# yynps737/zero-latency-yolo

Hardware: AMD Instinct MI355X
Metric: frames_per_sec (higher is better)
Workload: dtype bf16; 1 GPU; YOLOv8-nano 416x416 batch=64 throughput path (BASELINE configs[2]), bf16; engines_per_gpu=3, weights=seeded synthetic (no real weights offline), graph=True, parallelism=single GPU

## Files before the change

### zero-latency-yolo_amd/csrc/engine.cpp

```cpp
#include "zly_internal.h"
#include "weights.h"

#include <algorithm>
#include <atomic>
#include <chrono>
#include <condition_variable>
#include <deque>
#include <map>
#include <mutex>
#include <string>
#include <thread>
#include <type_traits>
#include <vector>
#include <string.h>
#include <stdio.h>
#include <stdlib.h>

namespace zly {

static thread_local std::string g_last_error;

static int fail(int code, const std::string& msg) { g_last_error = msg; return code; }

#define HIP_TRY(expr, code)                                                                        \
// ... 216 lines not shown
    num("ZLY_STEM1_TW", &sw->stem1_tw);
    num("ZLY_STEM1_TH", &sw->stem1_th);
    sw->stem1_keep_tiles = on("ZLY_STEM1_TW") || on("ZLY_STEM1_TH") || on("ZLY_STEM1_BIG_TILES");
    num("ZLY_PAIR_MIN_TILES", &sw->pair_min_tiles);
    num("ZLY_PAIR_WIDTHS", &sw->pair_widths);
    auto num_nonempty = [&](const char* name, int* out) { const char* v = getenv(name); if (v && *v) *out = atoi(v); };
    num_nonempty("ZLY_STAGE_SLOTS", &sw->stage_slots);
    num_nonempty("ZLY_STAGE_MB", &sw->stage_mb);
    num_nonempty("ZLY_INFLIGHT", &sw->inflight);
    { int d = 0; num_nonempty("ZLY_D2H_STREAM", &d); sw->d2h_stream = d != 0; }
    num("ZLY_PROFILE_INNER", &sw->profile_inner);
    if (sw->profile_inner < 1) sw->profile_inner = 1;
#ifdef ZLY_DIAG
    if (const char* v = getenv("ZLY_ABLATE_SKIP")) sw->ablate = std::string(",") + v + ",";
#endif
    sw->no_stream = on("ZLY_NO_STREAM");
    sw->stream_ct2 = on("ZLY_STREAM_CT2");
    num("ZLY_STREAM_MAX_NK", &sw->stream_max_nk);
    num("ZLY_STREAM_MIN_GROUPS", &sw->stream_min_groups);
    num("ZLY_STREAM_WGS", &sw->stream_wgs);
    num("ZLY_WS1", &sw->ws1_mode);
    sw->ws1_no_dual = on("ZLY_WS1_NO_DUAL");
    num("ZLY_WS1_MIN_PX", &sw->ws1_min_px);
    sw->ws1_max_bytes = on("ZLY_WS1_MAX_BYTES");
    sw->no_ws = on("ZLY_NO_WS");
    sw->no_ws_s2 = on("ZLY_NO_WS_S2");
    sw->no_ws_s2_c32 = on("ZLY_NO_WS_S2_C32");
    sw->ws_rowt = on("ZLY_WS_ROWT");
    num("ZLY_WS_TPW1_MAXCT", &sw->ws_tpw1_maxct);
    num("ZLY_WS_MIN_TILES", &sw->ws_min_tiles);
    num("ZLY_WS_MAX_BYTES", &sw->ws_max_bytes);
    num("ZLY_WS_PAIR", &sw->ws_pair);
    num("ZLY_WS_PAIR_GRID", &sw->ws_pair_grid);
    num("ZLY_WS_PAIR_MAX_TILES", &sw->ws_pair_max_tiles);
    sw->no_wres = on("ZLY_NO_WRES");
    num("ZLY_WRES_MAXCHUNKS", &sw->wres_maxchunks);
    sw->lds_s2_pt1 = on("ZLY_LDS_S2_PT1");
    num("ZLY_LDS_MIN_TILES", &sw->lds_min_tiles);
    num("ZLY_LDS_WGS_PER_CU", &sw->lds_wgs_per_cu);
    num("ZLY_DIRECT_PT4_MIN", &sw->direct_pt4_min);
    num("ZLY_DIRECT_PT2_MIN", &sw->direct_pt2_min);
    num("ZLY_DIRECT_KSPLIT_NK", &sw->direct_ksplit_nk);
    num("ZLY_C2F32_NW", &sw->c2f32_nw);
    num("ZLY_C2F_LDS_KB", &sw->c2f_lds_kb);
    if (const char* ft = getenv("ZLY_C2F_TILE")) { int th = 0, tw = 0; if (sscanf(ft, "%d,%d", &th, &tw) == 2) { sw->c2f_tile_th = th; sw->c2f_tile_tw = tw; } }
    sw->c2f64 = on("ZLY_C2F64");
}

struct PlanBuilder {
    Plan* p;
    const ModelFile& model;
    const zly_config& cfg;
    const int dtype;
    const Switches& sw;
    const size_t esz;
    const int kstep;
    std::string err;

    bool bf16() const { return dtype == ZLY_DTYPE_BF16; }
    bool fail(const std::string& msg) { err = msg; return false; }
    int add_buffer(const std::string& name, int H, int W, int C, bool f32 = false) {
        Buffer b;
        b.name = name; b.H = H; b.W = W; b.C = C; b.f32 = f32;
        p->bufs.push_back(b);
        return (int)p->bufs.size() - 1;
    }
// ... 2139 lines not shown
    const Op& op = e->ops[(size_t)i];
    std::string k;
    switch (L.kind) {
    case LK_NONE:
        switch (t[(size_t)L.covered_by].kind) {
        case LK_STEM: case LK_STEM1: k = op.kind == OP_PREPROCESS ? "(fused into stem_fused_kernel)" : "(fused into the previous launch)"; break;
        case LK_PAIR: case LK_WS_PAIR: k = "(fused into the previous launch)"; break;
        case LK_C2F: k = "(fused into the C2f kernel at " + e->ops[(size_t)L.covered_by].name + ")"; break;
        case LK_SPPF_FUSED: k = "(fused into the SPPF kernel at model.9.cv1)"; break;
        case LK_MULTI: k = "(in a merged Detect launch)"; break;
        case LK_HEAD: k = op.kind == OP_CONV ? "(computed in the Detect tail at surviving anchors)" : "(covered by the last tail launch)"; break;
        }
        break;
    case LK_PREPROCESS: k = L.lb ? "preprocess_kernel<LB> (letterbox)" : "preprocess_kernel"; break;
    case LK_STEM: k = L.lb ? "stem_fused_kernel<LB> (letterbox)" : "stem_fused_kernel"; break;
    case LK_STEM1: k = L.lb ? "stem_model1_kernel<LB> (letterbox preprocess+model.0+model.1)" : "stem_model1_kernel (preprocess+model.0+model.1)"; break;
    case LK_SPPF_POOL: k = L.pool16 ? "sppf_pool16_kernel<DPP row windows, one barrier>" : "sppf_pool_kernel"; break;
    case LK_SPPF_FUSED: k = "sppf_fused_kernel<cv1+3 pools+cv2,SPLIT=" + std::to_string(sppf_split(e->ops[(size_t)e->sppf_cv2].cout, n, e->sw)) + ">"; break;
    case LK_MULTI: k = L.multi_ct == 3 ? "conv_igemm_multi_kernel<CT=3> (the 3 Detect stems)" : "conv_igemm_multi_kernel<CT=2> (the 6 Detect branch convs)"; break;
    case LK_C2F: {
        const C2fGroup& g = e->c2fs[(size_t)op.c2f];
        k = "c2f_kernel<C=" + std::to_string(g.c) + (g.c == 32 ? ",NW=" + std::to_string(L.c2f.nw) : std::string()) +
            (g.mode == 3 ? ",cv1+bottleneck+cv2>" : g.mode == 1 ? ",cv1+bottleneck>" : ",bottleneck+cv2>");
        break;
    }
    case LK_PAIR: k = "bottleneck_pair_kernel<" + std::to_string(e->pairs[(size_t)op.pair].c) + ">"; break;
    case LK_WS_PAIR: k = std::string("conv3x3_ws_pair_kernel<") + (e->pairs[(size_t)op.pair].res ? "RES," : "") + "64->64->64," + std::to_string(L.ws_pair.g.TH) + "x" + std::to_string(L.ws_pair.g.TW) + " tiles>"; break;
    case LK_CONV_WSK: k = "conv3x3_wsk_kernel<K=720 packed across taps,5 channel tiles>"; break;
    case LK_CONV: {
        const int cin = op.in.C + (op.in2.buf >= 0 ? op.in2.C : 0);
        const ConvPlan& c = L.conv;
        switch (c.kind) {
        case CONV_WS1: k = std::string("conv1x1_ws_kernel<") + (op.in2.buf >= 0 ? "dual-source," : "") + "NK=" + std::to_string(cin / 32) + "," + std::to_string(c.ct) + " channel tiles," + std::to_string(c.pt * 16) + " px>"; break;
        case CONV_WS: k = std::string("conv3x3_ws_kernel<") + (op.stride == 2 ? "S=2," : "") + (c.rowt ? "ROWT," : "") + (c.tpw1 ? "TPW=1," : "TPW=2,") + std::to_string(c.ct) + " channel tiles>"; break;
        case CONV_LDS: k = "conv3x3_lds_kernel<S=" + std::to_string(op.stride) + ",CT=" + std::to_string(c.ct) + ",PT=" + std::to_string(c.pt) + (c.wres ? ",wres>" : ">"); break;
        case CONV_STREAM: k = "conv1x1_stream_kernel<CT=" + std::to_string(c.ct) + ",PT=" + std::to_string(c.pt) + ",NK=" + std::to_string((cin + 31) / 32) + ">"; break;
        default: k = std::string("conv_igemm_kernel<") + (op.ks == 1 ? (op.in2.buf >= 0 ? "1x1 dual-source" : "1x1") : (c.fastk ? "3x3" : "3x3 generic-K")) +
                 ",CT=" + std::to_string(c.ct) + ",PT=" + std::to_string(c.pt) + ",KSPLIT=" + std::to_string(c.ksplit) + ">";
        }
        break;
    }
    case LK_HEAD: {
        k = L.lb ? "head_fused_kernel<LB> (letterbox box mapping)" : "head_fused_kernel";
        std::string lv;
        for (int l = 0; l < 3; ++l)
            if (L.box_mode[l] && (L.only_level < 0 || L.only_level == l)) lv += std::string(lv.empty() ? "" : ",") + "P" + std::to_string(3 + l) + (L.box_mode[l] == 1 ? ":ws" : ":lds");
        if (!lv.empty()) k += " (+ box conv in k-step order " + lv + ")";
        break;
    }
    case LK_NMS: k = "nms_kernel"; break;
    }
    snprintf(out, cap, "%s", k.c_str());
    return ZLY_OK;
}

int32_t zly_launch_info_at(zly_engine* e, int32_t i, int32_t n, zly_launch_info* out)
{
    if (!e || !out || i < 0 || i >= (int32_t)e->ops.size() || n < 1 || n > e->cfg.max_batch) return fail(ZLY_ERR_INVALID_ARGUMENT, "bad argument");
    std::lock_guard<std::mutex> lk(e->mu);
    memset(out, 0, sizeof *out);
    const int nops = (int)e->ops.size();
    const std::vector<Launch>& t = resolve_launches(e, n);
    out->covered_by = t[(size_t)i].covered_by;
    if (out->covered_by != i) return ZLY_OK;
    std::vector<char> in_group((size_t)nops, 0);
    for (int j = 0; j < nops; ++j) in_group[(size_t)j] = t[(size_t)j].covered_by == i ? 1 : 0;
    std::map<int, std::vector<char>> written_in, read_out, counted_in, counted_out;
// ... 117 lines not shown
```

### zero-latency-yolo_amd/csrc/kernels_conv.hip

```cpp
#include "zly_internal.h"
#include "conv_device.h"
#include <type_traits>
#include <algorithm>

namespace zly {

template <int CT>
__device__ __forceinline__ void load_bias(const ConvArgs& a, int tile0, int kq, f32x4 (&bias)[CT])
{
    const int ntiles = (a.Cout + 15) >> 4;
    const int paired = (ntiles >> 1) << 1;
#pragma unroll
    for (int c = 0; c < CT; ++c) {
        const int ch = tile_channel(tile0 + c, kq, paired);
        bias[c] = ch < a.Cout ? *reinterpret_cast<const f32x4*>(a.bias + ch) : f32x4{0.f, 0.f, 0.f, 0.f};
    }
}

template <typename T, int CT>
__device__ __forceinline__ void epilogue_px(const ConvArgs& a, f32x4 (&v)[CT], const f32x4 (&bias)[CT], int tile0, int kq, int m)
{
    const int ntiles = (a.Cout + 15) >> 4;
    const int paired = (ntiles >> 1) << 1;
    f32x4 o[CT];
// ... 685 lines not shown
        for (int k = 0; k < 5; ++k) o[k] = dsum[k];
        o[5] = ditems; o[6] = __builtin_amdgcn_s_memtime() - dstart; o[7] = dsum[5];
    }
#endif
}

typedef void (*conv_lds_fn)(const ConvArgs, int, int, int, int);

template <int S, int PT>
static conv_lds_fn pick_lds_ct(int ct) {
    switch (ct) {
        case 2: return conv3x3_lds_kernel<S, 2, PT>;
        case 3: return conv3x3_lds_kernel<S, 3, PT>;
        case 4: return conv3x3_lds_kernel<S, 4, PT>;
        case 5: return conv3x3_lds_kernel<S, 5, PT>;
    }
    return nullptr;
}
static conv_lds_fn pick_lds(int stride, int pt, int ct) {
    if (stride == 1) return pt == 1 ? pick_lds_ct<1, 1>(ct) : pt == 2 ? pick_lds_ct<1, 2>(ct) : pick_lds_ct<1, 4>(ct);
    return pt == 1 ? pick_lds_ct<2, 1>(ct) : pick_lds_ct<2, 2>(ct);
}
static size_t lds_bytes(int stride, int pt, int ct, int wchunks = 1) {
    size_t patch = 0;
    if (stride == 1) patch = pt == 1 ? LdsGeom<1, 1>::PATCH_BYTES : pt == 2 ? LdsGeom<1, 2>::PATCH_BYTES : LdsGeom<1, 4>::PATCH_BYTES;
    else             patch = pt == 1 ? LdsGeom<2, 1>::PATCH_BYTES : LdsGeom<2, 2>::PATCH_BYTES;
    return patch + (size_t)wchunks * 9 * ct * 1024;
}

#ifdef ZLY_WS_DIAG
__device__ unsigned long long* g_ws_diag = nullptr;
#endif

template <int TPW, int NKS, bool RES, bool ROWT = false, int S = 1>
__global__ __launch_bounds__(256, 2) void conv3x3_ws_kernel(const ConvArgs a, const WsGeom g)
{
    extern __shared__ __attribute__((aligned(16))) unsigned char smem[];
    unsigned char* lpatch = smem;
    const int PW = S == 1 ? g.TW + 8 : g.TW + 8 * ((g.TW + 8) / 8), PH = S == 1 ? g.TH + 2 : 2 * g.TH + 1;
    const int PWV = S == 1 ? g.TW + 2 : 2 * g.TW + 1;
    static_assert(S == 1 || !ROWT, "row tiles: stride 1");
    const int nthreads = blockDim.x;
    const int tid = threadIdx.x, lane = tid & 63;
    const int wave = __builtin_amdgcn_readfirstlane(tid >> 6);
    const int p = lane & 15, kq = lane >> 4;
    const int wc = wave % g.nwc, wp = wave / g.nwc;
    const int ntiles_c = (a.cout_pad + 15) >> 4;
    const bf16_t* __restrict__ in = static_cast<const bf16_t*>(a.in) + a.in_co;
    const int upp = a.Cin >> 3;
    const int NPU = PH * PW * upp;
    const float inv_upp = 1.0f / (float)upp, invPW = 1.0f / (float)PW, invTW = 1.0f / (float)g.TW;
    const int NPB = g.TH * g.TW, nct = ROWT ? g.TH : (NPB + 15) >> 4;
    const int tiles_per_img = g.tiles_x * g.tiles_y;

    bf16x8 w[TPW][NKS];
    {
        const bf16_t* __restrict__ wb = static_cast<const bf16_t*>(a.wgt) + lane * 8;
#pragma unroll
        for (int t = 0; t < TPW; ++t) {
            const int tile = min(wc * TPW + t, ntiles_c - 1);
#pragma unroll
            for (int s = 0; s < NKS; ++s) w[t][s] = *reinterpret_cast<const bf16x8*>(wb + ((size_t)tile * a.nk + s) * 512);
        }
    }
    f32x4 biasr[TPW];
    load_bias<TPW>(a, wc * TPW, kq, biasr);
    const __amdgpu_buffer_rsrc_t rout = __builtin_amdgcn_make_buffer_rsrc(a.out, 0, (unsigned)((size_t)a.M * a.out_cs * 2), 0x00020000);
    const __amdgpu_buffer_rsrc_t rres = __builtin_amdgcn_make_buffer_rsrc(const_cast<void*>(a.res ? a.res : a.out), 0,
                                                                          (unsigned)((size_t)a.M * (a.res ? a.res_cs : a.out_cs) * 2), 0x00020000);
    const int ch0 = TPW == 2 ? wc * 32 + kq * 8 : tile_channel(wc, kq, (((a.Cout + 15) >> 4) >> 1) << 1);
    constexpr bool has_res = RES;
    int toff[NKS];
#pragma unroll
    for (int s = 0; s < NKS; ++s) {
        const int tap = s / (NKS / 9), chunk = s - tap * (NKS / 9);
        const int ky = tap / 3, kx = tap - ky * 3;
        toff[s] = (ky * PW + kx) * g.pitch + chunk * 64;
    }
#ifdef ZLY_WS_DIAG
    unsigned long long dsum[4] = {0, 0, 0, 0}, dT0 = 0, dT1 = 0;
#define WSSTAMP(t) do { __builtin_amdgcn_sched_barrier(0); asm volatile("s_memtime %0\n\ts_waitcnt lgkmcnt(0)" : "=s"(t) :: "memory"); __builtin_amdgcn_sched_barrier(0); } while (0)
#define WSPHASE(k) do { WSSTAMP(dT1); dsum[k] += dT1 - dT0; dT0 = dT1; } while (0)
    const unsigned long long dstart = __builtin_amdgcn_s_memtime();
    WSSTAMP(dT0);
#else
#define WSPHASE(k) do { } while (0)
#endif

    const int upitch = g.pitch >> 4;
    const int NLU = PH * PW * upitch, ndma = (NLU + 63) >> 6;
    const float inv_upitch = 1.0f / (float)upitch;
    const int patch_bytes = ndma * 1024;
    const __amdgpu_buffer_rsrc_t rin = __builtin_amdgcn_make_buffer_rsrc(const_cast<bf16_t*>(in), 0, (unsigned)(((size_t)a.M / (a.Ho * a.Wo) * a.H * a.W * a.in_cs - a.in_co) * 2), 0x00020000);
    auto dma_patch = [&](int tl, unsigned char* dst) {
        const int b = tl / tiles_per_img;
        const int r = tl - b * tiles_per_img;
        const int ty = r / g.tiles_x;
        const int y0 = ty * g.TH, x0 = (r - ty * g.tiles_x) * g.TW;
        for (int k = wave; k < ndma; k += nthreads >> 6) {
            const int u = k * 64 + lane;
            const int px = (int)(((float)u + 0.5f) * inv_upitch), part = u - px * upitch;
            const int py = (int)(((float)px + 0.5f) * invPW), pxx = px - py * PW;
            const int gy = y0 * S - 1 + py, gx = x0 * S - 1 + pxx;
            const bool ok = part < upp && pxx < PWV && py < PH && (unsigned)gy < (unsigned)a.H && (unsigned)gx < (unsigned)a.W;
            const unsigned off = ok ? (unsigned)((((b * a.H + gy) * a.W + gx) * a.in_cs) * 2 + part * 16) : 0x80000000u;
            __builtin_amdgcn_raw_ptr_buffer_load_lds(rin, (__attribute__((address_space(3))) void*)(dst + k * 1024), 16, off, 0, 0, 0);
        }
    };
    (void)NPU; (void)inv_upp; (void)patch_bytes;
    if ((int)blockIdx.x < g.total_tiles) dma_patch(blockIdx.x, lpatch);
    for (int tl = blockIdx.x; tl < g.total_tiles; tl += gridDim.x) {
        const int b = tl / tiles_per_img;
        const int r = tl - b * tiles_per_img;
        const int ty = r / g.tiles_x;
        const int y0 = ty * g.TH, x0 = (r - ty * g.tiles_x) * g.TW;
        unsigned char* cur = lpatch;
        asm volatile("s_waitcnt vmcnt(0)" ::: "memory");
        __syncthreads();
        WSPHASE(0);
        auto pair_setup = [&](int t0, const unsigned char* (&px)[2], int (&ob)[2], int (&rb)[2]) {
#pragma unroll
            for (int h2 = 0; h2 < 2; ++h2) {
                const int t = min(t0 + h2 * g.nwp, nct - 1);
                const int q = ROWT ? (p < g.TW ? t * g.TW + p : NPB) : t * 16 + p;
                const int qc = min(q, NPB - 1);
                const int oy = ROWT ? t : (int)(((float)qc + 0.5f) * invTW), ox = ROWT ? p : qc - oy * g.TW;
                px[h2] = cur + (oy * S * PW + ox * S) * g.pitch + kq * 16;
                const int gy = y0 + oy, gx = x0 + ox;
                const bool ok = (t0 + h2 * g.nwp < nct) && q < NPB && gy < a.Ho && gx < a.Wo;
                const int m = (b * a.Ho + gy) * a.Wo + gx;
                ob[h2] = ok ? (m * a.out_cs + a.out_co + ch0) * 2 : (int)0x80000000;
                rb[h2] = ok ? (m * a.res_cs + a.res_co + ch0) * 2 : (int)0x80000000;
            }
        };
        auto pair_mma = [&](const unsigned char* const (&px)[2], f32x4 (&acc)[2][TPW]) {
#pragma unroll
            for (int h2 = 0; h2 < 2; ++h2)
#pragma unroll
                for (int c = 0; c < TPW; ++c) acc[h2][c] = f32x4{0.f, 0.f, 0.f, 0.f};
            if constexpr (ROWT) {
                static_assert(!ROWT || NKS == 18, "row tiles: Cin = 64");
                bf16x8 xr[2][6];
#pragma unroll
// ... 70 lines not shown
                    if (has_res) {
                        const bf16x4 r = __builtin_bit_cast(bf16x4, __builtin_amdgcn_raw_buffer_load_b64(rres, rb[h2], 0, 0));
                        x += f32x4{(float)r[0], (float)r[1], (float)r[2], (float)r[3]};
                    }
                    const bf16x4 wv = to_bf16x4(x);
                    typedef __attribute__((ext_vector_type(2))) unsigned int u32x2;
                    __builtin_amdgcn_raw_buffer_store_b64(__builtin_bit_cast(u32x2, wv), rout, ob[h2], 0, 0);
                }
            }
        };
        if (wp < nct) {
            const unsigned char* pxa[2];
            int oba[2], rba[2];
            f32x4 acca[2][TPW];
            pair_setup(wp, pxa, oba, rba);
            pair_mma(pxa, acca);
            for (int t0 = wp + 2 * g.nwp; t0 < nct; t0 += 2 * g.nwp) {
                const unsigned char* pxb[2];
                int obb[2], rbb[2];
                f32x4 accb[2][TPW];
                pair_setup(t0, pxb, obb, rbb);
                pair_store(acca, oba, rba);
                pair_mma(pxb, accb);
#pragma unroll
                for (int h2 = 0; h2 < 2; ++h2) {
                    oba[h2] = obb[h2]; rba[h2] = rbb[h2];
#pragma unroll
                    for (int c = 0; c < TPW; ++c) acca[h2][c] = accb[h2][c];
                }
            }
            pair_store(acca, oba, rba);
        }
        WSPHASE(2);
        if (tl + (int)gridDim.x < g.total_tiles) {
            __syncthreads();
            dma_patch(tl + gridDim.x, lpatch);
        }
        WSPHASE(1);
    }
#ifdef ZLY_WS_DIAG
    if (lane == 0 && g_ws_diag) {
        unsigned long long* o = g_ws_diag + ((size_t)blockIdx.x * (blockDim.x >> 6) + wave) * 8;
        for (int k = 0; k < 3; ++k) o[k] = dsum[k];
        o[3] = __builtin_amdgcn_s_memtime() - dstart;
    }
#endif
}

__device__ __forceinline__ void ws_pair_mma(const bf16x8 (&w)[18], const unsigned char* const (&px)[2], const int (&toff)[18], f32x4 (&acc)[2])
{
    constexpr int WS_DEPTH = 3;
    acc[0] = f32x4{0.f, 0.f, 0.f, 0.f};
    acc[1] = f32x4{0.f, 0.f, 0.f, 0.f};
    bf16x8 xf[2][WS_DEPTH + 1];
#pragma unroll
    for (int s = 0; s < WS_DEPTH; ++s) { xf[0][s] = *reinterpret_cast<const bf16x8*>(px[0] + toff[s]); xf[1][s] = *reinterpret_cast<const bf16x8*>(px[1] + toff[s]); }
#pragma unroll
    for (int s = 0; s < 18; ++s) {
        if (s + WS_DEPTH < 18) {
            xf[0][(s + WS_DEPTH) % (WS_DEPTH + 1)] = *reinterpret_cast<const bf16x8*>(px[0] + toff[s + WS_DEPTH]);
            xf[1][(s + WS_DEPTH) % (WS_DEPTH + 1)] = *reinterpret_cast<const bf16x8*>(px[1] + toff[s + WS_DEPTH]);
        }
        acc[0] = mma_step(w[s], xf[0][s % (WS_DEPTH + 1)], acc[0]);
        acc[1] = mma_step(w[s], xf[1][s % (WS_DEPTH + 1)], acc[1]);
    }
}

constexpr int WS_PAIR_PATCH_MAX = 32 * 1024, WS_PAIR_MID_MAX = 32 * 1024;

template <bool RES>
__global__ __launch_bounds__(256, 2) void conv3x3_ws_pair_kernel(const WsPairArgs a, const WsPairGeom g)
{
    __shared__ __attribute__((aligned(16))) unsigned char lpatch[WS_PAIR_PATCH_MAX];
    __shared__ __attribute__((aligned(16))) unsigned char lmid[WS_PAIR_MID_MAX];
    constexpr int NKS = 18, PITCH = 160, UPITCH = PITCH / 16, UPP = 8;
    typedef __attribute__((ext_vector_type(2))) unsigned int u32x2;
    const int PWA = g.TW + 4, PHA = g.TH + 4;
// ... 343 lines not shown
            const long key = rounds * ((th * tw + 15) / 16 * 16 + 64) * 4096 + ph * pw;
            if (best < 0 || key < best) { best = key; g->TH = th; g->TW = tw; g->tiles_x = tx; g->tiles_y = ty; }
        }
    if (best < 0) return false;
    g->pitch = pitch; g->nchunks = 0;
    return true;
}

bool conv_wsk_ok(const ConvArgs& a, const Switches& sw, WskPlan* plan)
{
    if (a.Cin != 80 || a.Cout != 80 || a.nk != 23 || a.stride != 1 || a.pad != 1 || a.in2 || a.res || a.out_f32 || !a.act || a.in_cs % 8 || a.in_co % 8 || a.out_cs % 4 || a.out_co % 4) return false;
    if ((size_t)a.M * (size_t)std::max(a.in_cs, a.out_cs) * 2 >= ((size_t)1 << 31)) return false;
    const int n = a.M / (a.Ho * a.Wo);
    WsGeom g{};
    if (!wsk_plan(a.Ho, a.Wo, a.Cin, n, sw.num_cus, &g)) return false;
    const double util = (double)a.Ho * a.Wo / ((double)g.tiles_x * g.tiles_y * g.TH * g.TW);
    if (util < 0.7 || (long)n * a.Ho * a.Wo < sw.ws_min_tiles * 169L) return false;
    g.total_tiles = g.tiles_x * g.tiles_y * n;
    g.nwc = 5; g.nwp = 1;
    plan->g = g;
    plan->lds = (unsigned)(((size_t)(g.TH + 2) * (g.TW + 8) * g.pitch + 1023) / 1024 * 1024);
    plan->gx = (unsigned)(g.total_tiles < 2 * sw.num_cus ? g.total_tiles : 2 * sw.num_cus);
    return true;
}

hipError_t launch_conv_wsk(const ConvArgs& a, const WskPlan& plan, hipStream_t s)
{
    if (a.Cin != 80 || a.nk != 23 || plan.gx < 1) return hipErrorInvalidValue;
    hipLaunchKernelGGL(conv3x3_wsk_kernel<23>, dim3(plan.gx), dim3(320), plan.lds, s, a, plan.g);
    return hipGetLastError();
}

typedef void (*conv_ws_fn)(const ConvArgs, const WsGeom);
static conv_ws_fn pick_ws(int cin, int tpw, bool res = false, bool rowt = false, int stride = 1)
{
    if (stride == 2) {
        if (res || rowt) return nullptr;
        if (tpw == 1) return cin == 64 ? conv3x3_ws_kernel<1, 18, false, false, 2> : nullptr;
        if (tpw != 2) return nullptr;
        return cin == 64 ? conv3x3_ws_kernel<2, 18, false, false, 2> : cin == 32 ? conv3x3_ws_kernel<2, 9, false, false, 2> : nullptr;
    }
    if (cin != 64) return nullptr;
    if (rowt && tpw == 2) return res ? conv3x3_ws_kernel<2, 18, true, true> : conv3x3_ws_kernel<2, 18, false, true>;
    if (res) return tpw == 2 ? conv3x3_ws_kernel<2, 18, true> : conv3x3_ws_kernel<1, 18, true>;
    return tpw == 2 ? conv3x3_ws_kernel<2, 18, false> : conv3x3_ws_kernel<1, 18, false>;
}
static constexpr int WS_LDS_MAX = 64 * 1024;

static bool ws_plan(int H, int W, int cin, int n, int ncu, WsGeom* g, int stride = 1)
{
    if (!pick_ws(cin, 2, false, false, stride)) return false;
    const int pitch = cin * 2 + (stride == 2 ? 16 : 32);
    long best = -1;
    for (int th = (stride == 2 ? 2 : 4); th <= 32; ++th)
        for (int tw = 8; tw <= 32; ++tw) {
            const long ph = stride == 2 ? 2 * th + 1 : th + 2, pw = stride == 2 ? tw + 8 * ((tw + 8) / 8) : tw + 8;
            const long lds = (ph * pw * pitch + 1023) / 1024 * 1024;
            if (lds > WS_LDS_MAX) continue;
            const int tx = (W + tw - 1) / tw, ty = (H + th - 1) / th;
            const long tiles = (long)tx * ty * n;
            const long rounds = (tiles + 2 * ncu - 1) / (2 * ncu);
            const long key = rounds * ((th * tw + 15) / 16 * 16 + 64) * 4096 + ph * pw;
            if (best < 0 || key < best) { best = key; g->TH = th; g->TW = tw; g->tiles_x = tx; g->tiles_y = ty; }
        }
    if (best < 0) return false;
    g->pitch = pitch; g->nchunks = cin / 32;
    return true;
}

static bool ws_pair_tiles(int H, int W, int n, int ncu, WsPairGeom* g, unsigned* lds)
{
    long best = -1;
    for (int th = 4; th <= 32; ++th)
        for (int tw = 8; tw <= 14; ++tw) {
            const long patch = ((long)(th + 4) * (tw + 4) * 160 + 1023) / 1024 * 1024, mid = (long)(th + 2) * (tw + 8) * 160;
            if (patch + 1024 > WS_PAIR_PATCH_MAX || mid > WS_PAIR_MID_MAX) continue;
            const int tx = (W + tw - 1) / tw, ty = (H + th - 1) / th;
            const long tiles = (long)tx * ty * n;
            const long rounds = (tiles + 2 * ncu - 1) / (2 * ncu);
            const long key = rounds * ((th + 2) * 16 + (th * tw + 15) / 16 * 16 + 64) * 65536 + patch + mid;
            if (best < 0 || key < best) { best = key; g->TH = th; g->TW = tw; g->tiles_x = tx; g->tiles_y = ty; *lds = (unsigned)(WS_PAIR_PATCH_MAX + WS_PAIR_MID_MAX); }
        }
    return best >= 0;
}

typedef void (*conv_ws_pair_fn)(const WsPairArgs, const WsPairGeom);

bool conv_ws_pair_plan(const ConvArgs& a, const ConvArgs& b, const ConvPlan& pa, const ConvPlan& pb, const Switches& sw, WsPairPlan* plan)
{
    if (!sw.ws_pair || pa.kind != CONV_WS || pb.kind != CONV_WS) return false;
    if (pa.rowt || pb.rowt) return false;
// ... 17 lines not shown

hipError_t launch_conv_ws_pair(const ConvArgs& a, const ConvArgs& b, const WsPairPlan& plan, bool dump, hipStream_t s)
{
    if (!plan.fn || plan.gx < 1) return hipErrorInvalidValue;
    WsPairArgs pa{};
    pa.in = a.in; pa.in_cs = a.in_cs; pa.in_co = a.in_co;
    pa.wA = a.wgt; pa.bA = a.bias; pa.wB = b.wgt; pa.bB = b.bias;
    pa.H = a.H; pa.W = a.W; pa.n = a.M / (a.Ho * a.Wo);
    pa.out = b.out; pa.out_cs = b.out_cs; pa.out_co = b.out_co;
    pa.res = b.res; pa.res_cs = b.res_cs; pa.res_co = b.res_co;
    if (dump) { pa.mid = a.out; pa.mid_cs = a.out_cs; pa.mid_co = a.out_co; }
    hipLaunchKernelGGL(reinterpret_cast<conv_ws_pair_fn>(const_cast<void*>(plan.fn)), dim3(plan.gx), dim3(256), 0, s, pa, plan.g);
    return hipGetLastError();
}

hipError_t ws_init()
{
    {
        hipError_t r = hipFuncSetAttribute((const void*)conv3x3_wsk_kernel<23>, hipFuncAttributeMaxDynamicSharedMemorySize, WS_LDS_MAX);
        if (r != hipSuccess) return r;
    }
    for (int tpw = 1; tpw <= 2; ++tpw)
        for (int res = 0; res <= 1; ++res)
            for (int rowt = 0; rowt <= 1; ++rowt) {
                hipError_t r = hipFuncSetAttribute((const void*)pick_ws(64, tpw, res != 0, rowt != 0), hipFuncAttributeMaxDynamicSharedMemorySize, WS_LDS_MAX);
                if (r != hipSuccess) return r;
            }
    for (int cin = 32; cin <= 64; cin += 32) {
        hipError_t r = hipFuncSetAttribute((const void*)pick_ws(cin, 2, false, false, 2), hipFuncAttributeMaxDynamicSharedMemorySize, WS_LDS_MAX);
        if (r != hipSuccess) return r;
    }
    {
        hipError_t r = hipFuncSetAttribute((const void*)pick_ws(64, 1, false, false, 2), hipFuncAttributeMaxDynamicSharedMemorySize, WS_LDS_MAX);
        if (r != hipSuccess) return r;
    }
    return hipSuccess;
}

template <int TPW, int NK, bool DUAL = false>
__global__ __launch_bounds__(256, 2) void conv1x1_ws_kernel(const ConvArgs a, const Ws1Geom g)
{
    extern __shared__ __attribute__((aligned(16))) unsigned char smem[];
    const int tid = threadIdx.x, lane = tid & 63;
    const int wave = __builtin_amdgcn_readfirstlane(tid >> 6);
    const int p = lane & 15, kq = lane >> 4;
    const int wc = wave % g.nwc, wp = wave / g.nwc;
    const int tile0 = ((int)blockIdx.y * g.nwc + wc) * TPW;
    const bf16_t* __restrict__ in = static_cast<const bf16_t*>(a.in) + a.in_co;

    bf16x8 w[TPW][NK];
    {
        const bf16_t* __restrict__ wb = static_cast<const bf16_t*>(a.wgt) + lane * 8;
#pragma unroll
        for (int t = 0; t < TPW; ++t)
#pragma unroll
            for (int s = 0; s < NK; ++s) w[t][s] = *reinterpret_cast<const bf16x8*>(wb + ((size_t)(tile0 + t) * a.nk + s) * 512);
    }
    f32x4 biasr[TPW];
    load_bias<TPW>(a, tile0, kq, biasr);
    const __amdgpu_buffer_rsrc_t rout = __builtin_amdgcn_make_buffer_rsrc(a.out, 0, (unsigned)((size_t)a.M * a.out_cs * 2), 0x00020000);
    const __amdgpu_buffer_rsrc_t rin = __builtin_amdgcn_make_buffer_rsrc(const_cast<bf16_t*>(in), 0, (unsigned)(((size_t)(DUAL ? a.M >> 2 : a.M) * a.in_cs - a.in_co) * 2), 0x00020000);
    const __amdgpu_buffer_rsrc_t rin2 = __builtin_amdgcn_make_buffer_rsrc(const_cast<void*>(DUAL ? a.in2 : a.in), 0, (unsigned)((size_t)a.M * (DUAL ? a.in2_cs : a.in_cs) * 2), 0x00020000);
    const int ch0 = TPW == 2 ? (tile0 >> 1) * 32 + kq * 8 : tile_channel(tile0, kq, (((a.Cout + 15) >> 4) >> 1) << 1);

    const int upp = a.Cin >> 3, upitch = g.pitch >> 4;
    const int ndma = (g.npx * upitch + 63) >> 6;
// ... 329 lines not shown
    const int ntiles = a.cout_pad / 16;
    int ct = 0, pt = 0;
    if (nk <= 2 && ntiles == 2) { ct = 2; pt = 4; }
    else if (nk <= 4 && ntiles % 4 == 0) { ct = 4; pt = 2; }
    else if (nk == 6 && ntiles % 4 == 0 && !sw.stream_ct2) { ct = 4; pt = 1; }
    else if (nk == 8 && !sw.stream_ct2) return false;
    else if ((nk == 6 || nk == 8) && ntiles % 2 == 0) { ct = 2; pt = 1; }
    conv_stream_fn fn = ct ? pick_stream(ct, pt, nk) : nullptr;
    if (!fn || nk > sw.stream_max_nk) return false;
    if ((long)a.M / (16 * pt) * (ntiles / ct) < sw.stream_min_groups) return false;
    if (a.in2 || a.res || nk > a.nk || !a.act || a.out_f32 || a.Cout % 32 || a.in_cs % 8 || a.in_co % 8 || a.out_cs % 8 || a.out_co % 8) return false;
    *p = ConvPlan{};
    p->kind = CONV_STREAM; p->ct = ct; p->pt = pt; p->ksplit = 1;
    p->fn[0] = (const void*)fn;
    const int ytiles = a.cout_pad / (16 * ct);
    p->ngroups = (a.M + 16 * pt - 1) / (16 * pt);
    int gx = (p->ngroups + 3) / 4;
    const int wgs = sw.stream_wgs > 0 ? sw.stream_wgs : (ct == 4 && pt == 1 ? 2 : 4) * sw.num_cus;
    const int cap = wgs / ytiles > 0 ? wgs / ytiles : 1;
    if (gx > cap) gx = cap;
    p->gx = (unsigned)gx; p->gy = (unsigned)ytiles;
    return true;
}

static bool plan_ws(const ConvArgs& a, const Switches& sw, ConvPlan* p)
{
    const int stride = a.stride, cin = a.Cin, cout_pad = a.cout_pad, Ho = a.Ho, Wo = a.Wo, n = a.M / (a.Ho * a.Wo);
    const int ntiles = cout_pad / 16, even = ntiles / 2 * 2;
    if (sw.no_ws || cout_pad % 16 || (even != 2 && even != 4 && even != 8)) return false;
    if (stride == 2 && (ntiles != even || a.res || sw.no_ws_s2)) return false;
    if (stride == 2 && cin == 32 && ((long)n * Ho * Wo >= 200000 || sw.no_ws_s2_c32)) return false;
    if (stride != 1 && stride != 2) return false;
    if (a.pad != 1 || a.in2 || a.out_f32 || !a.act || a.nk != 9 * cin / 32 || a.in_cs % 8 || a.in_co % 8) return false;
    WsGeom g{};
    if (!ws_plan(Ho, Wo, cin, n, sw.num_cus, &g, stride)) return false;
    const double util = (double)Ho * Wo / ((double)g.tiles_x * g.tiles_y * g.TH * g.TW);
    if (util < 0.7 || (long)n * Ho * Wo < sw.ws_min_tiles * 169L) return false;
    const size_t widest = std::max(std::max((size_t)n * a.H * a.W * (size_t)a.in_cs, (size_t)a.M * (size_t)a.out_cs), a.res ? (size_t)a.M * (size_t)a.res_cs : (size_t)0) * 2;
    if (widest >= sw.ws_max_bytes) {
        if (!plan_lds(a, sw, p)) plan_direct(ZLY_DTYPE_BF16, 3, a, sw, p);
        return true;
    }
    *p = ConvPlan{};
    p->kind = CONV_WS; p->ct = ntiles; p->pt = 4; p->ksplit = 1; p->fastk = 1;
    p->rowt = (stride == 1 && sw.ws_rowt && g.TW + 2 <= 16) ? 1 : 0;
    p->tpw1 = (cin == 64 && cout_pad == 64 && (g.TH * g.TW + 15) / 16 <= sw.ws_tpw1_maxct) ? 1 : 0;
    g.total_tiles = g.tiles_x * g.tiles_y * n;
    p->lds = (unsigned)(stride == 2 ? ((size_t)(2 * g.TH + 1) * (g.TW + 8 * ((g.TW + 8) / 8)) * g.pitch + 1023) / 1024 * 1024
                                    : ((size_t)(g.TH + 2) * (g.TW + 8) * g.pitch + 1023) / 1024 * 1024);
    p->gx = (unsigned)(g.total_tiles < 2 * sw.num_cus ? g.total_tiles : 2 * sw.num_cus);
    p->gy = 1;
    const bool res = a.res != nullptr;
    if (p->tpw1) {
        g.nwc = 4; g.nwp = 1; p->tiles0 = ntiles;
        p->fn[0] = (const void*)(stride == 2 ? pick_ws(cin, 1, false, false, 2) : pick_ws(cin, 1, res));
    } else {
        g.nwc = even / 2; g.nwp = 4 / g.nwc; p->tiles0 = even;
        p->fn[0] = (const void*)(stride == 2 ? pick_ws(cin, 2, false, false, 2) : pick_ws(cin, 2, res, p->rowt != 0));
        if (stride == 1 && ntiles > even && a.Cout > even * 16) p->fn[1] = (const void*)pick_ws(cin, 1, res);
    }
    p->ws = g;
    return true;
}

static bool plan_ws1(const ConvArgs& a, const Switches& sw, ConvPlan* p)
{
    const bool dual = a.in2 != nullptr;
    Ws1Geom g{};
    int ny = 0;
    if (a.Cin < 128 || !ws1_plan(a.Cin, a.cout_pad, a.M, sw.num_cus, &g, &ny, dual) || a.M < sw.ws1_min_px) return false;
    if (a.stride != 1 || a.pad != 0 || a.res || !a.act || a.out_f32 || a.nk != a.Cin / 32 || a.Cout % 32 || a.cout_pad != a.Cout ||
        a.in_cs % 8 || a.in_co % 8 || a.out_cs % 8 || a.out_co % 8) return false;
    if (dual && (a.in2_cs % 8 || a.in2_co % 8 || a.split_c % 8 || a.split_c <= 0 || a.split_c >= a.Cin || (a.H & 1) || (a.W & 1) || a.M % (a.H * a.W))) return false;
    const size_t widest = (size_t)a.M * (size_t)std::max(std::max(a.in_cs, a.out_cs), dual ? a.in2_cs : 0) * 2;
    if (sw.ws1_max_bytes || widest >= ((size_t)1 << 31)) { plan_direct(ZLY_DTYPE_BF16, 1, a, sw, p); return true; }
    *p = ConvPlan{};
    p->kind = CONV_WS1; p->ct = a.cout_pad / 16; p->pt = g.npx / 16; p->ksplit = 1;
    p->fn[0] = (const void*)pick_ws1(ws1_tpw(a.nk), a.nk, dual);
    p->ws1 = g;
    p->lds = (unsigned)(((size_t)g.npx * g.pitch + 1023) / 1024 * 1024);
    int gx = 2 * sw.num_cus / ny;
    if (gx < 1) gx = 1;
    if (gx > g.total_tiles) gx = g.total_tiles;
    p->gx = (unsigned)gx; p->gy = (unsigned)ny;
    return true;
}

void conv_plan(int dtype, int ks, const ConvArgs& a, const Switches& sw, ConvPlan* p)
{
    const bool bf16 = dtype == ZLY_DTYPE_BF16, pointwise = bf16 && ks == 1 && a.stride == 1 && a.pad == 0;
    const bool streamable = !a.in2 && !a.res && a.act && !a.out_f32 && a.Cout % 32 == 0;
    if (a.in2 && ks == 1 && !a.res && a.act && !a.out_f32 && a.Cout % 32 == 0 && a.cout_pad == a.Cout) {
        if (pointwise && sw.ws1_mode > 0 && !sw.ws1_no_dual && plan_ws1(a, sw, p)) return;
        plan_direct(dtype, ks, a, sw, p);
        return;
    }
    const bool ws1_ok = pointwise && streamable && sw.ws1_mode > 0;
    if (ws1_ok && (sw.ws1_mode == 2 || a.M >= 131072) && plan_ws1(a, sw, p)) return;
    if (pointwise && streamable && !sw.no_stream && plan_stream(a, sw, p)) return;
    if (ws1_ok && plan_ws1(a, sw, p)) return;
    if (bf16 && ks == 3 && plan_ws(a, sw, p)) return;
    if (bf16 && ks == 3 && plan_lds(a, sw, p)) return;
    plan_direct(dtype, ks, a, sw, p);
}

hipError_t launch_conv(const ConvArgs& a, const ConvPlan& p, hipStream_t s)
{
    if (!p.fn[0] || p.gx < 1 || p.gy < 1) return hipErrorInvalidValue;
    const dim3 grid(p.gx, p.gy, 1);
    switch (p.kind) {
    case CONV_WS1:
        hipLaunchKernelGGL(reinterpret_cast<conv_ws1_fn>(const_cast<void*>(p.fn[0])), grid, dim3(256), p.lds, s, a, p.ws1);
        break;
    case CONV_WS: {
        ConvArgs m = a;
        m.cout_pad = p.tiles0 * 16;
        m.Cout = a.Cout < p.tiles0 * 16 ? a.Cout : p.tiles0 * 16;
        hipLaunchKernelGGL(reinterpret_cast<conv_ws_fn>(const_cast<void*>(p.fn[0])), grid, dim3(256), p.lds, s, m, p.ws);
        if (p.fn[1]) {
            ConvArgs r = a;
            r.wgt = static_cast<const char*>(a.wgt) + (size_t)p.tiles0 * a.nk * 1024;
            r.bias = a.bias + p.tiles0 * 16;
            r.out_co = a.out_co + p.tiles0 * 16;
            if (a.res) r.res_co = a.res_co + p.tiles0 * 16;
            r.Cout = a.Cout - p.tiles0 * 16; r.cout_pad = 16;
            WsGeom g = p.ws;
            g.nwc = 1; g.nwp = 4;
            hipLaunchKernelGGL(reinterpret_cast<conv_ws_fn>(const_cast<void*>(p.fn[1])), grid, dim3(256), p.lds, s, r, g);
        }
        break;
    }
    case CONV_LDS:
        hipLaunchKernelGGL(reinterpret_cast<conv_lds_fn>(const_cast<void*>(p.fn[0])), grid, dim3(256), p.lds, s, a, p.tiles_x, p.tiles_per_img, p.total_tiles, p.wres);
        break;
    case CONV_STREAM:
        hipLaunchKernelGGL(reinterpret_cast<conv_stream_fn>(const_cast<void*>(p.fn[0])), grid, dim3(256), 0, s, a, p.ngroups);
        break;
    case CONV_DIRECT: {
        ConvArgs b = a;
        b.inv_wo = 1.0f / (float)a.Wo; b.inv_ho = 1.0f / (float)a.Ho;
        hipLaunchKernelGGL(reinterpret_cast<conv_fn>(const_cast<void*>(p.fn[0])), grid, dim3(256), 0, s, b);
        break;
    }
    default:
        return hipErrorInvalidValue;
    }
    return hipGetLastError();
}

}
// ... 1 lines not shown
```

### zero-latency-yolo_amd/csrc/zly_internal.h

```cpp
#pragma once
#include <hip/hip_runtime.h>
#include <stdint.h>
#include <stddef.h>
#include <string>
#include "zly.h"

namespace zly {

typedef __bf16 bf16_t;

struct FrameDesc {
    unsigned long long src_off;
    int w, h;
};
#define ZLY_DESC_FMT_SHIFT 56
__host__ __device__ __forceinline__ unsigned long long desc_pack(unsigned long long off, int fmt) { return off | ((unsigned long long)fmt << ZLY_DESC_FMT_SHIFT); }
__host__ __device__ __forceinline__ unsigned long long desc_off(unsigned long long v) { return v & ((1ull << ZLY_DESC_FMT_SHIFT) - 1); }
__host__ __device__ __forceinline__ int desc_fmt(unsigned long long v) { return (int)(v >> ZLY_DESC_FMT_SHIFT); }

struct ViewRec {
    unsigned long long off1, off2;
    int pitch0, pitch1, pitch2;
    int pad_;
};
// ... 41 lines not shown
    bool no_cin_pad = false;
    bool no_stem1 = false;
    int  stem1_nw = 0;
    int  stem1_var = 1;
    int  stem1_grid = 0;
    int  stem1_tw = 0, stem1_th = 0;
    bool stem1_keep_tiles = false;
    int  pair_min_tiles = 32;
    int  pair_widths = 48;
    int  stage_slots = 6;
    int  stage_mb = 0;
    int  inflight = 2;
    bool d2h_stream = false;
    int  profile_inner = 1;
    std::string ablate;
    bool no_stream = false;
    bool stream_ct2 = false;
    int  stream_max_nk = 1 << 30;
    long stream_min_groups = 4096;
    int  stream_wgs = 0;
    int  ws1_mode = 1;
    bool ws1_no_dual = false;
    long ws1_min_px = 2048;
    bool ws1_max_bytes = false;
    bool no_ws = false;
    bool no_ws_s2 = false;
    bool no_ws_s2_c32 = false;
    bool ws_rowt = false;
    int  ws_tpw1_maxct = 6;
    long ws_min_tiles = 64;
    size_t ws_max_bytes = (size_t)1 << 31;
    int  ws_pair = 1;
    int  ws_pair_max_tiles = 2;
    int  ws_pair_grid = 0;
    bool no_wres = false;
    int  wres_maxchunks = 1;
    bool lds_s2_pt1 = false;
    long lds_min_tiles = 384;
    int  lds_wgs_per_cu = 0;
    long direct_pt4_min = 1024, direct_pt2_min = 512;
    int  direct_ksplit_nk = 1 << 30;
    int  c2f32_nw = 0;
    int  c2f_lds_kb = 0;
    int  c2f_tile_th = 0, c2f_tile_tw = 0;
    bool c2f64 = false;
};

enum ConvKind { CONV_DIRECT, CONV_LDS, CONV_STREAM, CONV_WS, CONV_WS1 };
struct WsGeom { int TH, TW, tiles_x, tiles_y, total_tiles, pitch, nchunks, nwc, nwp; };
struct Ws1Geom { int npx, total_tiles, pitch, nwc, nwp; };
struct ConvPlan {
    int kind;
    int ct, pt, ksplit;
    int fastk;
    int wres, rowt, tpw1;
    const void* fn[2];
    unsigned gx, gy;
    unsigned lds;
    int tiles_x, tiles_per_img, total_tiles;
    int ngroups;
    int tiles0;
    WsGeom ws;
    Ws1Geom ws1;
};
void       conv_plan(int dtype, int ks, const ConvArgs& a, const Switches& sw, ConvPlan* plan);
hipError_t launch_conv(const ConvArgs& a, const ConvPlan& plan, hipStream_t s);
hipError_t conv_init();
struct WskPlan { WsGeom g; unsigned gx, lds; };
bool       conv_wsk_ok(const ConvArgs& a, const Switches& sw, WskPlan* plan);
hipError_t launch_conv_wsk(const ConvArgs& a, const WskPlan& plan, hipStream_t s);
int        conv_kstep(int dtype);
struct WsPairArgs {
    const void* in;  int in_cs, in_co;
    const void* wA;  const float* bA;
    const void* wB;  const float* bB;
    int H, W, n;
    void* out;       int out_cs, out_co;
    const void* res; int res_cs, res_co;
    void* mid;       int mid_cs, mid_co;
};
struct WsPairGeom { int TH, TW, tiles_x, tiles_y, total_tiles; };
struct WsPairPlan { WsPairGeom g; unsigned gx, lds; const void* fn; };
bool       conv_ws_pair_plan(const ConvArgs& a, const ConvArgs& b, const ConvPlan& pa, const ConvPlan& pb, const Switches& sw, WsPairPlan* plan);
hipError_t launch_conv_ws_pair(const ConvArgs& a, const ConvArgs& b, const WsPairPlan& plan, bool dump, hipStream_t s);

struct PairArgs {
    const void* in;  int in_cs, in_co;
    void* out;       int out_cs, out_co;
// ... 120 lines not shown
```

Baseline: 113,900 frames/s.

## Compute odd leftover channel tile inside the 3x3 WS conv launch

For stride-1 3x3 weight-stationary convs with 64 input channels and an odd number of 16-channel output tiles, the leftover tile was previously handled by a second TPW=1 kernel launch that re-streamed the input. The main pair kernel now preloads that tile's weights and bias into extra LDS and computes it from the already-resident input patch after the paired tiles. This removes one launch and one re-read of the input activation. In exchange it raises the LDS request, can shrink the spatial tile the planner picks, and adds per-tile work to the pair kernel. A grid-size cap knob is also added but defaults to off.

```diff
diff --git a/zero-latency-yolo_amd/csrc/engine.cpp b/zero-latency-yolo_amd/csrc/engine.cpp
--- a/zero-latency-yolo_amd/csrc/engine.cpp
+++ b/zero-latency-yolo_amd/csrc/engine.cpp
@@ -272,6 +272,8 @@
     num("ZLY_WS_MAX_BYTES", &sw->ws_max_bytes);
     num("ZLY_WS_PAIR", &sw->ws_pair);
     num("ZLY_WS_PAIR_GRID", &sw->ws_pair_grid);
+    num("ZLY_WS_ODD_INLINE", &sw->ws_odd_inline);
+    num("ZLY_WS_GRID", &sw->ws_grid);
     num("ZLY_WS_PAIR_MAX_TILES", &sw->ws_pair_max_tiles);
     sw->no_wres = on("ZLY_NO_WRES");
     num("ZLY_WRES_MAXCHUNKS", &sw->wres_maxchunks);
@@ -2477,7 +2479,7 @@
         const ConvPlan& c = L.conv;
         switch (c.kind) {
         case CONV_WS1: k = std::string("conv1x1_ws_kernel<") + (op.in2.buf >= 0 ? "dual-source," : "") + "NK=" + std::to_string(cin / 32) + "," + std::to_string(c.ct) + " channel tiles," + std::to_string(c.pt * 16) + " px>"; break;
-        case CONV_WS: k = std::string("conv3x3_ws_kernel<") + (op.stride == 2 ? "S=2," : "") + (c.rowt ? "ROWT," : "") + (c.tpw1 ? "TPW=1," : "TPW=2,") + std::to_string(c.ct) + " channel tiles>"; break;
+        case CONV_WS: k = std::string("conv3x3_ws_kernel<") + (op.stride == 2 ? "S=2," : "") + (c.rowt ? "ROWT," : "") + (c.tpw1 ? "TPW=1," : "TPW=2,") + std::to_string(c.ct) + (c.odd ? " channel tiles,odd last tile in-launch>" : " channel tiles>"); break;
         case CONV_LDS: k = "conv3x3_lds_kernel<S=" + std::to_string(op.stride) + ",CT=" + std::to_string(c.ct) + ",PT=" + std::to_string(c.pt) + (c.wres ? ",wres>" : ">"); break;
         case CONV_STREAM: k = "conv1x1_stream_kernel<CT=" + std::to_string(c.ct) + ",PT=" + std::to_string(c.pt) + ",NK=" + std::to_string((cin + 31) / 32) + ">"; break;
         default: k = std::string("conv_igemm_kernel<") + (op.ks == 1 ? (op.in2.buf >= 0 ? "1x1 dual-source" : "1x1") : (c.fastk ? "3x3" : "3x3 generic-K")) +
diff --git a/zero-latency-yolo_amd/csrc/kernels_conv.hip b/zero-latency-yolo_amd/csrc/kernels_conv.hip
--- a/zero-latency-yolo_amd/csrc/kernels_conv.hip
+++ b/zero-latency-yolo_amd/csrc/kernels_conv.hip
@@ -741,11 +741,12 @@
 __device__ unsigned long long* g_ws_diag = nullptr;
 #endif
 
-template <int TPW, int NKS, bool RES, bool ROWT = false, int S = 1>
+template <int TPW, int NKS, bool RES, bool ROWT = false, int S = 1, bool ODD = false>
 __global__ __launch_bounds__(256, 2) void conv3x3_ws_kernel(const ConvArgs a, const WsGeom g)
 {
     extern __shared__ __attribute__((aligned(16))) unsigned char smem[];
     unsigned char* lpatch = smem;
+    static_assert(!ODD || (TPW == 2 && !RES && !ROWT && S == 1), "in-launch odd tile: the plain stride-1 pair form");
     const int PW = S == 1 ? g.TW + 8 : g.TW + 8 * ((g.TW + 8) / 8), PH = S == 1 ? g.TH + 2 : 2 * g.TH + 1;
     const int PWV = S == 1 ? g.TW + 2 : 2 * g.TW + 1;
     static_assert(S == 1 || !ROWT, "row tiles: stride 1");
@@ -787,7 +788,7 @@
         toff[s] = (ky * PW + kx) * g.pitch + chunk * 64;
     }
 #ifdef ZLY_WS_DIAG
-    unsigned long long dsum[4] = {0, 0, 0, 0}, dT0 = 0, dT1 = 0;
+    unsigned long long dsum[5] = {0, 0, 0, 0, 0}, dT0 = 0, dT1 = 0;
 #define WSSTAMP(t) do { __builtin_amdgcn_sched_barrier(0); asm volatile("s_memtime %0\n\ts_waitcnt lgkmcnt(0)" : "=s"(t) :: "memory"); __builtin_amdgcn_sched_barrier(0); } while (0)
 #define WSPHASE(k) do { WSSTAMP(dT1); dsum[k] += dT1 - dT0; dT0 = dT1; } while (0)
     const unsigned long long dstart = __builtin_amdgcn_s_memtime();
@@ -818,6 +819,17 @@
     };
     (void)NPU; (void)inv_upp; (void)patch_bytes;
     if ((int)blockIdx.x < g.total_tiles) dma_patch(blockIdx.x, lpatch);
+    unsigned char* const lodd = smem + patch_bytes;
+    if constexpr (ODD) {
+        const __amdgpu_buffer_rsrc_t rwo = __builtin_amdgcn_make_buffer_rsrc(const_cast<char*>(static_cast<const char*>(a.wgt)) + (size_t)ntiles_c * a.nk * 1024, 0, NKS * 1024, 0x00020000);
+        for (int k = wave; k < NKS; k += nthreads >> 6)
+            __builtin_amdgcn_raw_ptr_buffer_load_lds(rwo, (__attribute__((address_space(3))) void*)(lodd + k * 1024), 16, (unsigned)(k * 1024 + lane * 16), 0, 0, 0);
+        if (wave == (NKS & 3)) {
+            const __amdgpu_buffer_rsrc_t rbo = __builtin_amdgcn_make_buffer_rsrc(const_cast<float*>(a.bias), 0, (unsigned)(((a.Cout + 3) & ~3) * 4), 0x00020000);
+            const int ch = ntiles_c * 16 + lane * 4;
+            __builtin_amdgcn_raw_ptr_buffer_load_lds(rbo, (__attribute__((address_space(3))) void*)(lodd + NKS * 1024), 16, lane < 4 && ch < a.Cout ? (unsigned)(ch * 4) : 0x80000000u, 0, 0, 0);
+        }
+    }
     for (int tl = blockIdx.x; tl < g.total_tiles; tl += gridDim.x) {
         const int b = tl / tiles_per_img;
         const int r = tl - b * tiles_per_img;
@@ -954,6 +966,61 @@
             pair_store(acca, oba, rba);
         }
         WSPHASE(2);
+        if constexpr (ODD) {
+            const int nw = nthreads >> 6;
+            const int cho = ntiles_c * 16 + kq * 4;
+            constexpr int NT = 3;
+            for (int t0 = wave; t0 < nct; t0 += NT * nw) {
+                int lo = lane * 16;
+                asm volatile("" : "+v"(lo));
+                const unsigned char* lw = lodd + lo;
+                const f32x4 bo = *reinterpret_cast<const f32x4*>(lodd + NKS * 1024 + kq * 16);
+                const unsigned char* px[NT];
+                int ob[NT];
+                f32x4 acc[NT];
+#pragma unroll
+                for (int h = 0; h < NT; ++h) {
+                    const int t = min(t0 + h * nw, nct - 1);
+                    const int q = t * 16 + p;
+                    const int qc = min(q, NPB - 1);
+                    const int oy = (int)(((float)qc + 0.5f) * invTW), ox = qc - oy * g.TW;
+                    px[h] = cur + (oy * PW + ox) * g.pitch + kq * 16;
+                    const int gy = y0 + oy, gx = x0 + ox;
+                    const bool ok = (t0 + h * nw < nct) && q < NPB && gy < a.Ho && gx < a.Wo;
+                    const int m = (b * a.Ho + gy) * a.Wo + gx;
+                    ob[h] = ok ? (m * a.out_cs + a.out_co + cho) * 2 : (int)0x80000000;
+                    acc[h] = f32x4{0.f, 0.f, 0.f, 0.f};
+                }
+                constexpr int DEPTH = 2;
+                bf16x8 xf[NT][DEPTH + 1], wf[DEPTH + 1];
+#pragma unroll
+                for (int s = 0; s < DEPTH; ++s) {
+                    wf[s] = *reinterpret_cast<const bf16x8*>(lw + s * 1024);
+#pragma unroll
+                    for (int h = 0; h < NT; ++h) xf[h][s] = *reinterpret_cast<const bf16x8*>(px[h] + toff[s]);
+                }
+#pragma unroll
+                for (int s = 0; s < NKS; ++s) {
+                    if (s + DEPTH < NKS) {
+                        wf[(s + DEPTH) % (DEPTH + 1)] = *reinterpret_cast<const bf16x8*>(lw + (s + DEPTH) * 1024);
+#pragma unroll
+                        for (int h = 0; h < NT; ++h) xf[h][(s + DEPTH) % (DEPTH + 1)] = *reinterpret_cast<const bf16x8*>(px[h] + toff[s + DEPTH]);
+                    }
+#pragma unroll
+                    for (int h = 0; h < NT; ++h) acc[h] = mma_step(wf[s % (DEPTH + 1)], xf[h][s % (DEPTH + 1)], acc[h]);
+                }
+#pragma unroll
+                for (int h = 0; h < NT; ++h) {
+                    f32x4 o = acc[h] + bo;
+#pragma unroll
+                    for (int r2 = 0; r2 < 4; ++r2) o[r2] = silu<bf16_t>(o[r2]);
+                    const bf16x4 wv = to_bf16x4(o);
+                    typedef __attribute__((ext_vector_type(2))) unsigned int u32x2;
+                    __builtin_amdgcn_raw_buffer_store_b64(__builtin_bit_cast(u32x2, wv), rout, ob[h], 0, 0);
+                }
+            }
+            WSPHASE(3);
+        }
         if (tl + (int)gridDim.x < g.total_tiles) {
             __syncthreads();
             dma_patch(tl + gridDim.x, lpatch);
@@ -965,6 +1032,7 @@
         unsigned long long* o = g_ws_diag + ((size_t)blockIdx.x * (blockDim.x >> 6) + wave) * 8;
         for (int k = 0; k < 3; ++k) o[k] = dsum[k];
         o[3] = __builtin_amdgcn_s_memtime() - dstart;
+        o[4] = dsum[3];
     }
 #endif
 }
@@ -1374,8 +1442,9 @@
 }
 
 typedef void (*conv_ws_fn)(const ConvArgs, const WsGeom);
-static conv_ws_fn pick_ws(int cin, int tpw, bool res = false, bool rowt = false, int stride = 1)
-{
+static conv_ws_fn pick_ws(int cin, int tpw, bool res = false, bool rowt = false, int stride = 1, bool odd = false)
+{
+    if (odd) return (cin == 64 && tpw == 2 && !res && !rowt && stride == 1) ? conv3x3_ws_kernel<2, 18, false, false, 1, true> : nullptr;
     if (stride == 2) {
         if (res || rowt) return nullptr;
         if (tpw == 1) return cin == 64 ? conv3x3_ws_kernel<1, 18, false, false, 2> : nullptr;
@@ -1388,8 +1457,9 @@
     return tpw == 2 ? conv3x3_ws_kernel<2, 18, false> : conv3x3_ws_kernel<1, 18, false>;
 }
 static constexpr int WS_LDS_MAX = 64 * 1024;
-
-static bool ws_plan(int H, int W, int cin, int n, int ncu, WsGeom* g, int stride = 1)
+static constexpr int WS_ODD_W_BYTES = 19 * 1024, WS_ODD_LDS_MAX = 72 * 1024;
+
+static bool ws_plan(int H, int W, int cin, int n, int ncu, WsGeom* g, int stride = 1, int lds_max = WS_LDS_MAX)
 {
     if (!pick_ws(cin, 2, false, false, stride)) return false;
     const int pitch = cin * 2 + (stride == 2 ? 16 : 32);
@@ -1398,7 +1468,7 @@
         for (int tw = 8; tw <= 32; ++tw) {
             const long ph = stride == 2 ? 2 * th + 1 : th + 2, pw = stride == 2 ? tw + 8 * ((tw + 8) / 8) : tw + 8;
             const long lds = (ph * pw * pitch + 1023) / 1024 * 1024;
-            if (lds > WS_LDS_MAX) continue;
+            if (lds > lds_max) continue;
             const int tx = (W + tw - 1) / tw, ty = (H + th - 1) / th;
             const long tiles = (long)tx * ty * n;
             const long rounds = (tiles + 2 * ncu - 1) / (2 * ncu);
@@ -1482,6 +1552,10 @@
     }
     {
         hipError_t r = hipFuncSetAttribute((const void*)pick_ws(64, 1, false, false, 2), hipFuncAttributeMaxDynamicSharedMemorySize, WS_LDS_MAX);
+        if (r != hipSuccess) return r;
+    }
+    {
+        hipError_t r = hipFuncSetAttribute((const void*)pick_ws(64, 2, false, false, 1, true), hipFuncAttributeMaxDynamicSharedMemorySize, WS_ODD_LDS_MAX);
         if (r != hipSuccess) return r;
     }
     return hipSuccess;
@@ -1877,8 +1951,10 @@
     if (stride == 2 && cin == 32 && ((long)n * Ho * Wo >= 200000 || sw.no_ws_s2_c32)) return false;
     if (stride != 1 && stride != 2) return false;
     if (a.pad != 1 || a.in2 || a.out_f32 || !a.act || a.nk != 9 * cin / 32 || a.in_cs % 8 || a.in_co % 8) return false;
+    const bool odd = stride == 1 && ntiles > even && a.Cout > even * 16;
+    const bool odd_inline = odd && sw.ws_odd_inline && !sw.ws_rowt && !a.res && pick_ws(cin, 2, false, false, 1, true);
     WsGeom g{};
-    if (!ws_plan(Ho, Wo, cin, n, sw.num_cus, &g, stride)) return false;
+    if (!ws_plan(Ho, Wo, cin, n, sw.num_cus, &g, stride, odd_inline ? WS_ODD_LDS_MAX - WS_ODD_W_BYTES : WS_LDS_MAX)) return false;
     const double util = (double)Ho * Wo / ((double)g.tiles_x * g.tiles_y * g.TH * g.TW);
     if (util < 0.7 || (long)n * Ho * Wo < sw.ws_min_tiles * 169L) return false;
     const size_t widest = std::max(std::max((size_t)n * a.H * a.W * (size_t)a.in_cs, (size_t)a.M * (size_t)a.out_cs), a.res ? (size_t)a.M * (size_t)a.res_cs : (size_t)0) * 2;
@@ -1894,6 +1970,7 @@
     p->lds = (unsigned)(stride == 2 ? ((size_t)(2 * g.TH + 1) * (g.TW + 8 * ((g.TW + 8) / 8)) * g.pitch + 1023) / 1024 * 1024
                                     : ((size_t)(g.TH + 2) * (g.TW + 8) * g.pitch + 1023) / 1024 * 1024);
     p->gx = (unsigned)(g.total_tiles < 2 * sw.num_cus ? g.total_tiles : 2 * sw.num_cus);
+    if (sw.ws_grid > 0 && p->gx > (unsigned)sw.ws_grid) p->gx = (unsigned)sw.ws_grid;
     p->gy = 1;
     const bool res = a.res != nullptr;
     if (p->tpw1) {
@@ -1902,7 +1979,10 @@
     } else {
         g.nwc = even / 2; g.nwp = 4 / g.nwc; p->tiles0 = even;
         p->fn[0] = (const void*)(stride == 2 ? pick_ws(cin, 2, false, false, 2) : pick_ws(cin, 2, res, p->rowt != 0));
-        if (stride == 1 && ntiles > even && a.Cout > even * 16) p->fn[1] = (const void*)pick_ws(cin, 1, res);
+        if (odd_inline) {
+            p->fn[0] = (const void*)pick_ws(cin, 2, false, false, 1, true);
+            p->odd = 1; p->lds += WS_ODD_W_BYTES;
+        } else if (odd) p->fn[1] = (const void*)pick_ws(cin, 1, res);
     }
     p->ws = g;
     return true;
@@ -1960,7 +2040,7 @@
     case CONV_WS: {
         ConvArgs m = a;
         m.cout_pad = p.tiles0 * 16;
-        m.Cout = a.Cout < p.tiles0 * 16 ? a.Cout : p.tiles0 * 16;
+        m.Cout = p.odd || a.Cout < p.tiles0 * 16 ? a.Cout : p.tiles0 * 16;
         hipLaunchKernelGGL(reinterpret_cast<conv_ws_fn>(const_cast<void*>(p.fn[0])), grid, dim3(256), p.lds, s, m, p.ws);
         if (p.fn[1]) {
             ConvArgs r = a;
diff --git a/zero-latency-yolo_amd/csrc/zly_internal.h b/zero-latency-yolo_amd/csrc/zly_internal.h
--- a/zero-latency-yolo_amd/csrc/zly_internal.h
+++ b/zero-latency-yolo_amd/csrc/zly_internal.h
@@ -97,6 +97,8 @@
     size_t ws_max_bytes = (size_t)1 << 31;
     int  ws_pair = 1;
     int  ws_pair_max_tiles = 2;
+    int  ws_odd_inline = 1;
+    int  ws_grid = 0;
     int  ws_pair_grid = 0;
     bool no_wres = false;
     int  wres_maxchunks = 1;
@@ -119,6 +121,7 @@
     int ct, pt, ksplit;
     int fastk;
     int wres, rowt, tpw1;
+    int odd;
     const void* fn[2];
     unsigned gx, gy;
     unsigned lds;
```

New measurement: 114,800 frames/s, median of 6. Within noise of the previous version (+0.8%).
